# hediet/slideo

Hardware: AMD Instinct MI355X
Metric: frames/sec matched (1080p vs 500-page ORB set) (higher is better)
Workload: dtype u8

## Files before the change

### slideo_amd/csrc/capi_runtime.hip

```cpp
#include "runtime.hpp"
#include <chrono>

using namespace slideo;

namespace slideo {

namespace {
std::string g_create_error;
std::mutex g_err_mutex;
}

void check_launch(const char* what) {
    hipError_t e = hipGetLastError();
    if (e != hipSuccess) fail(SLIDEO_ERR_HIP, "launch of %s failed: %s", what, hipGetErrorString(e));
}

GeomEntry& geom_for(slideo_matcher* m, int w, int h) {
    for (auto& g : m->geoms) if (g->w == w && g->h == h) return *g;
    if (w < 1 || h < 1 || w > MAX_DIM || h > MAX_DIM)
        fail(SLIDEO_ERR_UNSUPPORTED, "image size %dx%d outside 1..%d", w, h, MAX_DIM);
    auto e = std::make_unique<GeomEntry>();
    e->w = w; e->h = h;
    std::vector<uint32_t> tab;
    build_pyr_geom(w, h, m->cfg, e->g, tab);
// ... 224 lines not shown
    const PyrGeom& g = geom_for(m, f.w, f.h).g;
    const uint32_t kpcap = kp_cap_for(m, g);
    const bool async = allow_async && m->async_submit && !knn_unit_is_valu(m) &&
                       (int64_t)n * kpcap < ((int64_t)1 << 30) &&
                       (kpcap >= (uint32_t)c.nfeatures + 1024u || kpcap >= (uint32_t)std::max(g.cand_per_frame, 1));
    S.timed = prof; S.u_in = f; S.u_mask = mask_pyr; S.u_async = async;
    if (m->orb_chain && m->last_orb_ev && m->last_orb_ev != S.ev_orb) HIP_CHECK(hipStreamWaitEvent(st, m->last_orb_ev, 0));
    if (prof) HIP_CHECK(hipEventRecord(S.ev[0], st));
    orb_stage1(m, S, f, n, false, async ? kpcap : 0xFFFFFFFFu, mask_pyr);
    uint32_t qtot, qplan;
    if (async) {
        qtot = (uint32_t)n * kpcap;
        qplan = (uint32_t)n * std::min<uint32_t>(kpcap, (uint32_t)c.nfeatures);
        S.orb.qtot = qtot; S.orb.max_count = kpcap;
    } else {
        orb_wait_info(m, S);
        qtot = qplan = S.orb.qtot;
    }
    knn_plan_unit(m, S, n, (int64_t)f.w * f.h, qplan, qtot);
    S.d_votes.reserve(std::max<size_t>((size_t)qtot * c.knn_k * sizeof(uint2), 16));
    S.d_gpts.reserve(std::max<size_t>((size_t)qtot * c.knn_k * sizeof(float4), 16));
    S.d_gmask.reserve(std::max<size_t>((size_t)qtot * c.knn_k, 16));
    S.d_fcs.reserve((size_t)n * sizeof(FrameCands));
    S.d_verdicts.reserve((size_t)n * sizeof(slideo_verdict));
    S.d_pairs.reserve((size_t)n * MAXR * sizeof(PairDesc) + 64);
    S.h_out.reserve((size_t)n * (sizeof(slideo_verdict) + sizeof(FrameCands)) + 64);
    orb_stage2(m, S, f.w, f.h, async);
    HIP_CHECK(hipEventRecord(S.ev_orb, st));
    m->last_orb_ev = S.ev_orb;
    VerifyParams vp = make_vp(c);
    vp.rng_len = m->rng_len;
    HIP_CHECK(hipMemsetAsync(S.d_fcs.p, 0, (size_t)n * sizeof(FrameCands), st));
    if (prof) HIP_CHECK(hipEventRecord(S.ev[1], st));
    if (qtot > 0) unit_knn(m, S, n, qplan, qtot, async, prof);
    unit_verify(m, S, vp, f, n, qtot);
}

void unit_collect(slideo_matcher* m, Slot& S, slideo_verdict* out_host) {
    const int n = S.n;
    HIP_CHECK(hipStreamSynchronize(S.st));
    S.busy = false;
    const uint8_t* ho = S.h_out.as<uint8_t>();
    const size_t tail = (size_t)n * (sizeof(slideo_verdict) + sizeof(FrameCands));
    uint32_t fl, info[2];
    std::memcpy(&fl, ho + tail, 4);
    std::memcpy(info, ho + tail + 4, 8);
    if (S.u_async) {
        if (fl & 1u) fail(SLIDEO_ERR_HIP, "internal: FAST candidate list overflow");
        if (fl & 8u) {
            S.u_rerun = true;
            unit_submit(m, S, S.u_in, n, S.u_mask, false);
            unit_collect(m, S, out_host);
            return;
        }
        S.orb.qtot = info[0]; S.orb.max_count = info[1];
    }
    const uint32_t qtot = S.orb.qtot;
    if (fl & 4u) {
        const uint32_t cap = 1u << 26;
        if (m->rng_len >= cap) fail(SLIDEO_ERR_CAPACITY, "RANSAC sample schedule exceeded %u pre-drawn RNG outputs", m->rng_len);
        HIP_CHECK(hipDeviceSynchronize());
        upload_rng_stream(m, (uint32_t)std::min<uint64_t>((uint64_t)m->rng_len * 4, cap));
        S.u_rerun = true;
        unit_submit(m, S, S.u_in, n, S.u_mask, false);
        unit_collect(m, S, out_host);
        return;
    }
    if (S.timed) {
// ... 1078 lines not shown
```

### slideo_amd/csrc/capi_taps.hip

```cpp
#include "runtime.hpp"

using namespace slideo;

extern "C" {


int32_t slideo_orb_bgr8(slideo_matcher* m, const uint8_t* bgr, int32_t width, int32_t height, int32_t stride_bytes,
                        slideo_keypoint* kp, uint8_t* desc32, int32_t capacity, int32_t* n_out) {
    if (!m) return SLIDEO_ERR_INVALID_ARG;
    API_TRY
    if (!bgr || !n_out) fail(SLIDEO_ERR_INVALID_ARG, "null image/n_out");
    FrameSrc img = FrameSrc::image(bgr, width, height, stride_bytes);
    validate_frames(img);
    HIP_CHECK(hipSetDevice(m->device));
    require_idle(m);
    Slot& S = m->slots[0];
    hipStream_t st = S.st;
    const uint8_t* mask_pyr = (m->fs.mask.set && width == m->fs.mask.w && height == m->fs.mask.h) ? frame_mask_for(m, width, height) : nullptr;
    run_orb(m, S, stage_frames(m, S, img, 0, 1), 1, false, false, mask_pyr);
    const uint32_t q = S.orb.qtot;
    *n_out = (int32_t)q;
    if ((int64_t)q > capacity) fail(SLIDEO_ERR_CAPACITY, "%u keypoints, capacity %d", q, capacity);
    if (q) {
        if (kp) HIP_CHECK(hipMemcpyAsync(kp, S.d_kp.p, (size_t)q * sizeof(slideo_keypoint), hipMemcpyDeviceToHost, st));
// ... 119 lines not shown
    Slot& S = m->slots[0];
    hipStream_t st = S.st;
    const size_t tail = (size_t)n * (sizeof(slideo_verdict) + sizeof(FrameCands));
    for (;;) {
        S.knn.shared = false; S.gate.on = false; S.u_set = m->cur_set; S.u_rerun = false;
        const DevFrames f = stage_frames(m, S, src, 0, n);
        S.timed = false; S.u_in = f; S.u_mask = nullptr; S.u_async = false;
        S.orb.qofs = qofs; S.orb.qtot = qtot; S.orb.max_count = mx; S.orb.nframes = n;
        S.d_kp.reserve(std::max<size_t>((size_t)qtot * sizeof(slideo_keypoint), 16));
        S.d_desc.reserve(std::max<size_t>((size_t)qtot * 32, 32));
        S.d_qofs.reserve((size_t)(n + 1) * 4 + 16); S.d_info.reserve(64); S.d_flags.reserve(16);
        S.h_info.reserve((size_t)(n + 1) * 4 + 16);
        uint32_t* hq = S.h_info.as<uint32_t>();
        std::memcpy(hq, qofs.data(), (size_t)(n + 1) * 4);
        hq[n + 1] = qtot; hq[n + 2] = mx;
        if (qtot > 0) {
            HIP_CHECK(hipMemcpyAsync(S.d_kp.p, kp, (size_t)qtot * sizeof(slideo_keypoint), hipMemcpyHostToDevice, st));
            HIP_CHECK(hipMemcpyAsync(S.d_desc.p, desc32, (size_t)qtot * 32, hipMemcpyHostToDevice, st));
        }
        HIP_CHECK(hipMemcpyAsync(S.d_qofs.p, hq, (size_t)(n + 1) * 4, hipMemcpyHostToDevice, st));
        HIP_CHECK(hipMemcpyAsync(S.d_info.p, hq + n + 1, 8, hipMemcpyHostToDevice, st));
        HIP_CHECK(hipMemsetAsync(S.d_flags.p, 0, 16, st));
        knn_plan_unit(m, S, n, (int64_t)f.w * f.h, qtot, qtot);
        S.d_votes.reserve(std::max<size_t>((size_t)qtot * c.knn_k * sizeof(uint2), 16));
        S.d_gpts.reserve(std::max<size_t>((size_t)qtot * c.knn_k * sizeof(float4), 16));
        S.d_gmask.reserve(std::max<size_t>((size_t)qtot * c.knn_k, 16));
        S.d_fcs.reserve((size_t)n * sizeof(FrameCands));
        S.d_verdicts.reserve((size_t)n * sizeof(slideo_verdict));
        S.d_pairs.reserve((size_t)n * MAXR * sizeof(PairDesc) + 64);
        S.h_out.reserve(tail + 64);
        HIP_CHECK(hipMemsetAsync(S.d_fcs.p, 0, (size_t)n * sizeof(FrameCands), st));
        VerifyParams vp = make_vp(c);
        vp.rng_len = m->rng_len;
        if (qtot > 0) unit_knn(m, S, n, qtot, qtot, false, false);
        unit_verify(m, S, vp, f, n, qtot);
        HIP_CHECK(hipStreamSynchronize(st));
        S.busy = false;
        uint32_t fl;
        std::memcpy(&fl, S.h_out.as<uint8_t>() + tail, 4);
        if (!(fl & 4u)) break;
        const uint32_t cap = 1u << 26;
        if (m->rng_len >= cap) fail(SLIDEO_ERR_CAPACITY, "RANSAC sample schedule exceeded %u pre-drawn RNG outputs", m->rng_len);
        HIP_CHECK(hipDeviceSynchronize());
        upload_rng_stream(m, (uint32_t)std::min<uint64_t>((uint64_t)m->rng_len * 4, cap));
    }
    const uint8_t* ho = S.h_out.as<uint8_t>();
    std::memcpy(verdicts_out, ho, (size_t)n * sizeof(slideo_verdict));
    m->last_fcs.resize((size_t)n);
    std::memcpy(m->last_fcs.data(), ho + (size_t)n * sizeof(slideo_verdict), (size_t)n * sizeof(FrameCands));
    API_CATCH(m)
}

int32_t slideo_yuv420_to_bgr8(slideo_matcher* m, const uint8_t* frame, int32_t width, int32_t height, const slideo_yuv420_layout* layout,
                              uint8_t* bgr_out, int64_t out_capacity) {
    if (!m) return SLIDEO_ERR_INVALID_ARG;
    API_TRY
    if (!frame || !bgr_out) fail(SLIDEO_ERR_INVALID_ARG, "null frame/bgr_out");
    FrameSrc img = FrameSrc::yuv420(frame, false, width, height, layout, -1);
    img.describe(m->fs);
    img.levels = false;
    validate_frames(img);
    const size_t fb = (size_t)width * height * 3;
    if ((int64_t)fb > out_capacity) fail(SLIDEO_ERR_CAPACITY, "the BGR image needs %zu bytes", fb);
    tap_staged(m, img, bgr_out, (int64_t)fb);
    API_CATCH(m)
}

}
// ... 1 lines not shown
```

### slideo_amd/csrc/orb.hip.h

```cpp
#pragma once
#include <limits.h>
#include <hip/hip_runtime.h>
#include <stdint.h>

#include "geom.h"
#include "types.h"
#include "cv_math.hip.h"

namespace slideo {

__global__ __launch_bounds__(256) void gray_kernel(const uint8_t* __restrict__ frames, int64_t frame_stride,
                                                   int stride, uint8_t* __restrict__ pyr, int64_t pyr_frame_bytes,
                                                   int w, int h, int pitch, int aligned4, GrayCoef gc) {
    const uint32_t half = 1u << (gc.shift - 1);
    auto gray_of = [&](uint32_t b, uint32_t g, uint32_t r) { return (__umul24(b, gc.cb) + __umul24(g, gc.cg) + __umul24(r, gc.cr) + half) >> gc.shift; };
    const int x = (blockIdx.x * 256 + threadIdx.x) * 4;
    const int y = blockIdx.y;
    if (x >= w) return;
    const uint8_t* src = frames + (int64_t)blockIdx.z * frame_stride + (int64_t)y * stride + (int64_t)x * 3;
    uint8_t* dst = pyr + (int64_t)blockIdx.z * pyr_frame_bytes + (int64_t)y * pitch + x;
    if (aligned4 && x + 3 < w) {
        const uint32_t* s = reinterpret_cast<const uint32_t*>(src);
        uint32_t a = s[0], b = s[1], c = s[2];
        uint32_t g0 = gray_of(a & 255, (a >> 8) & 255, (a >> 16) & 255);
// ... 63 lines not shown
#pragma unroll
            for (int i = 0; i < 4; ++i) {
                const int xo = xe[i] & 0xffff, cx1 = xe[i] >> 16, cx0 = 256 - cx1;
                const int xo1 = min(xo + 1, src.w - 1);
                uint32_t h0 = (uint32_t)cx0 * r0[xo] + (uint32_t)cx1 * r0[xo1];
                uint32_t h1 = (uint32_t)cx0 * r1[xo] + (uint32_t)cx1 * r1[xo1];
                v[i] = (uint32_t)cy0 * h0 + (uint32_t)cy1 * h1 + (1u << 15);
            }
        }
        const uint32_t outv = __builtin_amdgcn_perm(__builtin_amdgcn_perm(v[3], v[2], 0x0c0c0602u),
                                                    __builtin_amdgcn_perm(v[1], v[0], 0x0c0c0602u), 0x05040100u);
        uint8_t* d = base + dst.ofs + __umul24(y, dst.pitch) + x0;
        if (nx == 4) *reinterpret_cast<uint32_t*>(d) = outv;
        else for (int i = 0; i < nx; ++i) d[i] = (uint8_t)(outv >> (8 * i));
    }
}

__global__ __launch_bounds__(256) void resize_quad_kernel(uint8_t* __restrict__ pyr, int64_t pyr_frame_bytes,
                                                          LevelGeom src, LevelGeom dst,
                                                          const uint32_t* __restrict__ lin_tab, int nxq, uint32_t nxq_magic) {
    const uint32_t t = blockIdx.x * 256 + threadIdx.x;
    const uint32_t yg = nxq_magic ? __umulhi(t, nxq_magic) : t;
    const uint32_t y0 = yg * 4u;
    if ((int)y0 >= dst.h) return;
    const uint32_t q = t - __umul24(yg, (uint32_t)nxq);
    const uint8_t* __restrict__ sbase = pyr + (int64_t)blockIdx.z * pyr_frame_bytes + src.ofs;
    uint8_t* __restrict__ dbase = pyr + (int64_t)blockIdx.z * pyr_frame_bytes + dst.ofs;
    const uint4 sel4 = reinterpret_cast<const uint4*>(lin_tab + dst.xsel_ofs)[q];
    const uint4 cp4 = reinterpret_cast<const uint4*>(lin_tab + dst.xctab_ofs)[q];
    const uint32_t xs = lin_tab[dst.xs_ofs + q];
    const uint4 ye4 = *reinterpret_cast<const uint4*>(lin_tab + dst.ytab_ofs + y0);
    const uint32_t ye[4] = {ye4.x, ye4.y, ye4.z, ye4.w};
    const uint32_t sel[4] = {sel4.x, sel4.y, sel4.z, sel4.w}, cp[4] = {cp4.x, cp4.y, cp4.z, cp4.w};
    uint2 a[4], b[4];
#pragma unroll
    for (int r = 0; r < 4; ++r) {
        const uint32_t yo = ye[r] & 0xffffu;
        const uint32_t o0 = __umul24(yo, (uint32_t)src.pitch) + xs;
        const uint32_t o1 = __umul24(min(yo + 1u, (uint32_t)(src.h - 1)), (uint32_t)src.pitch) + xs;
        {
            const uint32_t sh = (xs & 3u) * 8u;
            uint32_t w0[3], w1[3];
            __builtin_memcpy(w0, sbase + (o0 & ~3u), 12);
            __builtin_memcpy(w1, sbase + (o1 & ~3u), 12);
            a[r] = make_uint2(__builtin_amdgcn_alignbit(w0[1], w0[0], sh), __builtin_amdgcn_alignbit(w0[2], w0[1], sh));
            b[r] = make_uint2(__builtin_amdgcn_alignbit(w1[1], w1[0], sh), __builtin_amdgcn_alignbit(w1[2], w1[1], sh));
        }
    }
    const uint32_t dofs = __umul24(y0, (uint32_t)dst.pitch) + 4u * q;
#pragma unroll
    for (int r = 0; r < 4; ++r) {
        const uint32_t cy1 = ye[r] >> 16, cy0 = 256u - cy1;
        uint32_t v[4];
#pragma unroll
        for (int i = 0; i < 4; ++i) {
            const uint32_t ta = __builtin_amdgcn_perm(a[r].y, a[r].x, sel[i]);
            const uint32_t tb = __builtin_amdgcn_perm(b[r].y, b[r].x, sel[i]);
            v[i] = __umul24(cy0, dot2_u16(ta, cp[i])) + (__umul24(cy1, dot2_u16(tb, cp[i])) + (1u << 15));
        }
        const uint32_t outv = __builtin_amdgcn_perm(__builtin_amdgcn_perm(v[3], v[2], 0x0c0c0602u),
                                                    __builtin_amdgcn_perm(v[1], v[0], 0x0c0c0602u), 0x05040100u);
        if ((int)(y0 + r) < dst.h) *reinterpret_cast<uint32_t*>(dbase + (dofs + (uint32_t)r * (uint32_t)dst.pitch)) = outv;
    }
}

__device__ __forceinline__ bool run9(uint32_t m) {
    m |= m << 16;
    m &= m >> 1; m &= m >> 2; m &= m >> 4; m &= m >> 1;
    return m != 0;
}

__device__ __forceinline__ int level_of_tile(const PyrGeom& g, int tile, bool blur) {
    int l = 0;
    for (int i = 1; i < g.nlevels; ++i) {
        int t0 = blur ? g.lv[i].btile0 : g.lv[i].ftile0;
        int n = blur ? g.lv[i].btx * g.lv[i].bty : g.lv[i].ftx * g.lv[i].fty;
        if (n > 0 && tile >= t0) l = i;
    }
    return l;
}

constexpr int FAST_SW = FAST_TW + 2, FAST_SH = FAST_TH + 2;
constexpr int FAST_XO = 4;
constexpr int FAST_RW = FAST_TW + 14, FAST_RH = FAST_TH + 8;
static_assert(FAST_SW == 128 && FAST_RW % 4 == 0 && (FAST_RW / 4) % 2 == 1 && FAST_RW >= FAST_SW + FAST_XO + 3, "fast_kernel maps one score row onto two wave-widths");

typedef short fast_s2 __attribute__((ext_vector_type(2)));
typedef unsigned short fast_us2 __attribute__((ext_vector_type(2)));
__device__ __forceinline__ fast_s2 fast_swap(fast_s2 a) { return __builtin_shufflevector(a, a, 1, 0); }

#ifndef FAST_TPB_V
#define FAST_TPB_V 8
#endif
constexpr int FAST_TPB = FAST_TPB_V;
constexpr int FAST_STAGE_CAP = 128;
// ... 873 lines not shown
```

### slideo_amd/csrc/runtime.hpp

```cpp
#pragma once
#include <hip/hip_runtime.h>

#include <algorithm>
#include <cmath>
#include <cstdlib>
#include <functional>
#include <map>
#include <memory>
#include <mutex>
#include <string>
#include <vector>

#include "common.h"
#include "frame_settings.h"
#include "geom.h"
#include "slideo_amd.h"
#include "types.h"

namespace slideo {

#ifndef SLIDEO_NSLOTS
#define SLIDEO_NSLOTS 4
#endif
constexpr int NSLOTS = SLIDEO_NSLOTS;
// ... 339 lines not shown
    float max_error = std::sqrt((255.0f * 255.0f * 3.0f) * (float)n);
    return 1.0f - (float)e / max_error;
}
uint8_t* stage_for_upload(slideo_matcher* m, Slot& S, size_t bytes);
void tap_staged(slideo_matcher* m, const FrameSrc& img, uint8_t* out, int64_t ob);
void analyse_pages(slideo_matcher* m, int n_pages, const uint8_t* const* data, const int32_t* width, const int32_t* height, const int32_t* stride_bytes,
                   std::vector<HostPage>& out, uint64_t progress_base, uint64_t progress_total);
void append_page(slideo_matcher* m, const HostPage& pg);

void orb_stage_init(slideo_matcher* m);
void orb_geom_init(slideo_matcher* m, GeomEntry& e, const std::vector<uint32_t>& lin_tab);
void orb_stage1(slideo_matcher* m, Slot& S, const DevFrames& f, int n, bool with_blur = false, uint32_t kp_cap = 0xFFFFFFFFu,
                const uint8_t* mask_pyr = nullptr);
void orb_wait_info(slideo_matcher* m, Slot& S);
void orb_stage2(slideo_matcher* m, Slot& S, int w, int h, bool by_capacity = false);
void run_orb(slideo_matcher* m, Slot& S, const DevFrames& f, int n, bool keep_host_qofs, bool with_blur = false, const uint8_t* mask_pyr = nullptr);
void frame_mask_build(slideo_matcher* m, const uint8_t* mask, int w, int h, int stride, DevBuf& out);
const uint8_t* frame_mask_for(const slideo_matcher* m, int w, int h);
void orb_launch_gray(const slideo_matcher* m, const uint8_t* frames_dev, int64_t frame_stride, int stride, uint8_t* gray, int64_t gframe, int w, int h,
                     int pitch, int n, hipStream_t st);
void orb_launch_scan(const uint32_t* counts, int n, uint32_t* qofs, uint32_t* info, hipStream_t st);
void launch_reduce(slideo_matcher* m, const uint8_t* src, int64_t src_fs, int stride, int w, int h, int dw, int dh, int n, uint8_t* dst,
                   hipStream_t st);
void launch_rectify(const FrameRegion& R, const uint8_t* src, int64_t src_fs, int stride, int n, uint8_t* dst, hipStream_t st);
void frame_region_classify(FrameRegion& R);
void launch_yuv420_to_bgr(const YuvDesc& desc, const uint8_t* src, int64_t src_fs, const slideo_yuv420_layout& L, int w, int h, int n, uint8_t* dst, hipStream_t st,
                          const uint32_t* transfer_tab = nullptr);
void launch_pixels_to_bgr(int format, const uint8_t* src, int64_t src_fs, int stride, int w, int h, int n, uint8_t* dst, hipStream_t st);
void launch_levels(slideo_matcher* m, const uint8_t* src, int64_t src_fs, int src_stride, uint8_t* dst, int64_t dst_fs, int dst_stride, int w, int h,
                   int n, hipStream_t st);

void knn_build_index(slideo_matcher* m, const std::vector<uint8_t>& train, int64_t M);
void knn_plan_unit(slideo_matcher* m, Slot& S, int n, int64_t frame_pixels, uint32_t qplan, uint32_t qtot);
void unit_knn(slideo_matcher* m, Slot& S, int n, uint32_t qplan, uint32_t qtot, bool async, bool prof);
bool knn_unit_is_valu(const slideo_matcher* m);
void knn_expand_operand(const uint32_t* t, int nt, int nt_pad, const int32_t* perm, uint4* tx, hipStream_t st);
int knn_operand_rows(int nt);
OperandLayout knn_operand_layout();
std::vector<int32_t> knn_tile_order(int ntiles);
void l2_prepare(slideo_matcher::L2Set& L, const uint8_t* t, int nt, hipStream_t st);
void l2_query(slideo_matcher* m, slideo_matcher::L2Set& L, const uint8_t* q_dev, int nq, int k, hipStream_t st, Slot& S, bool timed,
              DevBuf* keys = nullptr, DevBuf* pend = nullptr, float prune_tol = 0.f);
void l2_lists_to_keys(slideo_matcher* m, Slot& S, const DevBuf& lists, int kq, uint32_t qtot, bool lowe, hipStream_t st);

void verify_stage_init(slideo_matcher* m);
VerifyParams make_vp(const slideo_config& c);
void unit_verify(slideo_matcher* m, Slot& S, const VerifyParams& vp, const DevFrames& f, int n, uint32_t qtot);
void run_small(slideo_matcher* m, const DevFrames& imgs, int n, hipStream_t st, int* sw = nullptr, int* sh = nullptr);
void run_small_into(slideo_matcher* m, const DevFrames& imgs, int n, DevBuf& dst, hipStream_t st, int* sw = nullptr, int* sh = nullptr);
void launch_ssd(const uint8_t* a, int64_t a_stride, const uint8_t* b, int64_t b_stride, int64_t bytes, unsigned long long* ssd, int n, hipStream_t st);

int page_set_create(slideo_matcher* m, int n, const int32_t* pages);
const PageSet* page_set_of(const slideo_matcher* m, int set);
void page_set_check_mode(const slideo_matcher* m);

void gate_release(slideo_matcher* m);
inline void gate_state_reset(slideo_matcher* m) { m->gate = slideo_matcher::GateState{}; }
inline size_t gate_small_budget(const slideo_matcher* m) {
    const size_t small = (size_t)m->cfg.small_area * 3 + 64;
    const size_t settle = m->fs.settle_similarity > 0.f ? small + 256 + 32 : 0;
    const size_t M = (size_t)m->fs.gate_memory;
    const size_t memory = M > 0 ? 8 * M + 8 : 0;
    const size_t anchor = m->fs.gate_ref == SLIDEO_GATE_ANCHOR ? small + 128 + 32 + (size_t)GATE_ANCHOR_MAX_UNIT * 8 + settle + memory : 0;
    if (!(m->fs.direct_t > 0.f)) return small + anchor;
    const size_t look = 2 * small + 128 + m->pages.size() * 8 + 64 + anchor;
    return m->fs.direct_scope == SLIDEO_DIRECT_VALID ? look + m->pages.size() * 8 : look;
}
inline size_t gate_memory_budget(const slideo_matcher* m) {
    const size_t M = m->fs.gate_ref == SLIDEO_GATE_ANCHOR ? (size_t)m->fs.gate_memory : 0;
    return M > 0 ? (M + 64) * ((size_t)m->cfg.small_area * 3 + 64 + 128) + 2048 : 0;
}
void gate_check(const slideo_matcher::GateState& g, const FrameSrc& src);
void gate_prime(slideo_matcher* m, FrameSrc src, hipStream_t user_stream);
void gate_state_read(slideo_matcher* m, hipEvent_t behind, size_t sb, uint8_t* anchor, uint8_t* prev, uint32_t* d);
void gate_state_write(slideo_matcher* m, size_t sb, const uint8_t* anchor, const uint8_t* prev, const uint32_t* d, hipStream_t st);
inline void gate_chain_receive(slideo_matcher* m, hipStream_t st) {
    if (!m->gate_receive) return;
    const std::function<void(hipStream_t)> f = std::move(m->gate_receive);
    m->gate_receive = nullptr;
    f(st);
// ... 64 lines not shown
```

### slideo_amd/csrc/stage_knn.hip

```cpp
#include "runtime.hpp"
#include "knn.hip.h"
#include "knn_tile.hip.h"
#include "knn_l2.hip.h"
#include "knn_lsh.hip.h"

using namespace slideo;

namespace slideo {

int knn_operand_rows(int nt) { return cdiv(std::max(nt, 1), KT_ST_ROWS) * KT_ST_ROWS; }
OperandLayout knn_operand_layout() { return OperandLayout{KT_ST_ROWS, KT_SIDE_U32, KT_PAD_NORM}; }

void knn_expand_operand(const uint32_t* t, int nt, int nt_pad, const int32_t* perm, uint4* tx, hipStream_t st) {
    knn_tile_expand_kernel<<<cdiv(nt_pad * 8, 256), 256, 0, st>>>(t, nt, nt_pad, perm, tx);
    check_launch("knn_tile_expand_kernel");
}

std::vector<int32_t> knn_tile_order(int ntiles) {
    std::vector<int32_t> order((size_t)ntiles);
    for (int i = 0; i < ntiles; ++i) order[i] = i;
    uint64_t st_ = 0x9E3779B97F4A7C15ull;
    for (int i = ntiles - 1; i > 0; --i) {
        st_ = st_ * 6364136223846793005ull + 1442695040888963407ull;
        std::swap(order[i], order[(int)((st_ >> 33) % (uint64_t)(i + 1))]);
// ... 156 lines not shown
    const uint4* tx = op.tx.as<uint4>(); const uint32_t* side = op.side.as<uint32_t>(); const float4* nminh = op.bound.as<float4>();
    const int nt_pad = knn_operand_rows(p.nt);
    uint32_t *keys = S.d_keys.as<uint32_t>(), *pend = S.d_knn_pend.as<uint32_t>();
    unsigned long long* const clk = m->profiling ? m->d_clk.as<unsigned long long>() : nullptr;
    if (lsh)
        knn_tile2_lsh_kernel<<<grid, KT_THREADS, 0, st>>>(q_dev, nq, tx, side, nminh, nt_pad, p.per_seg, keys, pend, prune_tol, nq_dev, *lsh);
    else if (p.engine == 2)
        knn_tile4_kernel<<<grid, KT_THREADS, 0, st>>>(q_dev, nq, tx, side, nminh, nt_pad, p.per_seg, keys, pend, prune_tol, nq_dev);
    else if (p.shape == SHAPE_T2W12)
        knn_tile2w12_kernel<<<grid, KT_WAVES12 * 64, 0, st>>>(q_dev, nq, tx, side, nminh, nt_pad, p.per_seg, keys, pend, prune_tol, nq_dev, clk);
    else
        knn_tile2_kernel<<<grid, KT_THREADS, p.lds_pad, st>>>(q_dev, nq, tx, side, nminh, nt_pad, p.per_seg, keys, pend, prune_tol, nq_dev, clk);
    check_launch(lsh ? "knn_tile2_lsh_kernel" : "knn_tile_kernel");
    if (p.nseg > 1) {
        knn_merge_kernel<KLIST><<<cdiv(p.nq_all, KNN_BLOCK), KNN_BLOCK, 0, st>>>(keys, nq, p.nseg, nq_dev);
        check_launch("knn_merge_kernel");
    }
}

static void run_knn(slideo_matcher* m, Slot& S, const KnnPlan& p, const uint32_t* q_dev, int nq, const uint32_t* t, const SearchOperand& op,
                    float prune_tol, const uint32_t* nq_dev = nullptr) {
    if (nq <= 0 && !nq_dev) return;
    if ((int64_t)p.nt >= ((int64_t)1 << KNN_KEY_SHIFT)) fail(SLIDEO_ERR_UNSUPPORTED, "train set of %d rows exceeds %d", p.nt, 1 << KNN_KEY_SHIFT);
    if (p.engine != 1) { knn_launch_tiles(m, S, p, q_dev, nq, op, prune_tol, nq_dev); return; }
    if (nq_dev) fail(SLIDEO_ERR_STATE, "internal: the VALU kNN engine needs the query count on the host");
    knn_hamming_kernel<KLIST><<<dim3(p.qblocks, p.nseg), KNN_BLOCK, 0, S.st>>>(q_dev, nq, t, p.nt, p.per_seg, S.d_keys.as<uint32_t>());
    check_launch("knn_hamming_kernel");
    if (p.nseg > 1) {
        knn_merge_kernel<KLIST><<<p.qblocks, KNN_BLOCK, 0, S.st>>>(S.d_keys.as<uint32_t>(), nq, p.nseg);
        check_launch("knn_merge_kernel");
    }
}

void unit_knn(slideo_matcher* m, Slot& S, int n, uint32_t qplan, uint32_t qtot, bool async, bool prof) {
    const slideo_config& c = m->cfg;
    hipStream_t st = S.st;
    const KnnPlan& p = S.knn;
    const PageSet* ps = page_set_of(m, S.u_set);
    const SearchOperand& op = ps ? ps->op : m->train_op;
    const uint32_t* nqd = async ? S.d_qofs.as<uint32_t>() + n : nullptr;
    const float prune = (m->knn_exact_lists || m->cfg.ratio_test > 0.f) ? 0.f : std::max(m->cfg.vote_tolerance, 1.0f);
    if (c.matcher == 1 && (m->lsh_gather || knn_unit_is_valu(m))) {
        knn_lsh_kernel<KLIST><<<cdiv((int)std::max(qtot, 1u), 4), 256, 0, st>>>(m->lsh.dev, S.d_desc.as<uint32_t>(), (int)qtot, m->d_train.as<uint32_t>(),
                                                                               S.d_keys.as<uint32_t>(), nqd);
        check_launch("knn_lsh_kernel");
    } else if (c.matcher == 1) {
        S.d_qkeys.reserve(std::max<size_t>((size_t)qtot * c.lsh_tables * 2, 64));
        lsh_query_keys_kernel<<<cdiv((int)std::max(qtot, 1u), 256), 256, 0, st>>>(m->lsh.dev.p, S.d_desc.as<uint32_t>(), (int)qtot, S.d_qkeys.as<uint16_t>(), nqd);
        check_launch("lsh_query_keys_kernel");
        const KtLshCtx ctx{m->lsh.dev.keys, S.d_qkeys.as<uint16_t>(), c.lsh_tables, c.lsh_multi_probe};
        knn_launch_tiles(m, S, p, S.d_desc.as<uint32_t>(), (int)qplan, op, prune, nqd, &ctx);
    } else
        run_knn(m, S, p, S.d_desc.as<uint32_t>(), (int)qplan, ps ? nullptr : m->d_train.as<uint32_t>(), op, prune, nqd);
    if (prof) HIP_CHECK(hipEventRecord(S.ev[2], st));
    if (p.dedup) {
        knn_expand_dups_kernel<KLIST><<<cdiv((int)std::max(qtot, 1u), KNN_BLOCK), KNN_BLOCK, 0, st>>>(
            S.d_keys.as<uint32_t>(), (int)qtot, (ps ? ps->d_grp_next : m->d_grp_next).as<int32_t>(), nqd);
        check_launch("knn_expand_dups_kernel");
    }
}

void knn_build_index(slideo_matcher* m, const std::vector<uint8_t>& train, int64_t M) {
    m->d_train.reserve(std::max<size_t>(train.size(), 64) + 64);
    HIP_CHECK(hipMemcpy(m->d_train.p, train.data(), train.size(), hipMemcpyHostToDevice));
    std::vector<int32_t> order((size_t)M), grp_next((size_t)M, -1), urow;
    for (int64_t i = 0; i < M; ++i) order[i] = (int32_t)i;
    m->Mu = M;
    if (m->cfg.matcher == 1) build_lsh_set(m->cfg, train.data(), (int)M, m->lsh, m->stream);
    if (m->knn_dedup && m->cfg.matcher == 0) {
        const uint64_t* t64 = reinterpret_cast<const uint64_t*>(train.data());
        auto less = [&](int32_t a, int32_t b) {
            const uint64_t* x = t64 + (size_t)a * 4; const uint64_t* y = t64 + (size_t)b * 4;
            for (int j = 0; j < 4; ++j) if (x[j] != y[j]) return x[j] < y[j];
            return a < b;
        };
        std::sort(order.begin(), order.end(), less);
        std::vector<uint8_t> head((size_t)M, 1);
        for (int64_t i = 1; i < M; ++i)
            if (std::memcmp(t64 + (size_t)order[i - 1] * 4, t64 + (size_t)order[i] * 4, 32) == 0) { grp_next[order[i - 1]] = order[i]; head[order[i]] = 0; }
        for (int64_t i = 0; i < M; ++i) if (head[i]) urow.push_back((int32_t)i);
        m->Mu = (int64_t)urow.size();
    }
    m->d_grp_next.reserve(grp_next.size() * 4 + 16);
    HIP_CHECK(hipMemcpy(m->d_grp_next.p, grp_next.data(), grp_next.size() * 4, hipMemcpyHostToDevice));
    if (m->Mu < M) {
        std::vector<uint8_t> utrain((size_t)m->Mu * 32);
        for (int64_t i = 0; i < m->Mu; ++i) std::memcpy(utrain.data() + (size_t)i * 32, train.data() + (size_t)urow[i] * 32, 32);
        m->d_utrain.reserve(utrain.size() + 64);
        HIP_CHECK(hipMemcpy(m->d_utrain.p, utrain.data(), utrain.size(), hipMemcpyHostToDevice));
        prepare_train_bits(utrain.data(), m->d_utrain.as<uint32_t>(), (int)m->Mu, m->train_op, m->stream, urow.data(), &m->h_uorder);
        m->h_urow.swap(urow);
    } else {
// ... 185 lines not shown
```

### slideo_amd/csrc/stage_sift.hip

```cpp
#include "runtime.hpp"
#include "sift.hip.h"

using namespace slideo;

namespace slideo {

static SiftGeom sift_geom(int w, int h) {
    SiftGeom g{};
    g.w = w; g.h = h;
    int bw = 2 * w, bh = 2 * h;
    g.n_oct = std::max(0, (int)std::lrint(std::log((double)std::min(bw, bh)) / std::log(2.) - 2) + 1);
    if (g.n_oct > SIFT_MAX_OCT) g.n_oct = SIFT_MAX_OCT;
    int64_t go = 0, dofs = 0;
    for (int o = 0; o < g.n_oct; ++o) {
        g.ow[o] = bw; g.oh[o] = bh; g.g_ofs[o] = go; g.d_ofs[o] = dofs;
        go += (int64_t)bw * bh * (SIFT_NL + 3); dofs += (int64_t)bw * bh * (SIFT_NL + 2);
        bw /= 2; bh /= 2;
        if (bw < 1 || bh < 1) { g.n_oct = o + 1; break; }
    }
    g.g_frame = go; g.d_frame = dofs;
    return g;
}

static SiftTaps sift_taps(double sigma) {
// ... 215 lines not shown
    S.orb.qtot = qtot; S.orb.max_count = mx; S.orb.nframes = n;
    S.knn.nt = (int)m->M;
    S.d_qofs.reserve((size_t)(n + 1) * 4 + 16); S.d_info.reserve(16); S.d_flags.reserve(16);
    S.h_info.reserve((size_t)(n + 1) * 4 + 16);
    uint32_t* hq = S.h_info.as<uint32_t>();
    std::memcpy(hq, S.orb.qofs.data(), (size_t)(n + 1) * 4);
    hq[n + 1] = qtot; hq[n + 2] = mx;
    HIP_CHECK(hipMemcpyAsync(S.d_qofs.p, hq, (size_t)(n + 1) * 4, hipMemcpyHostToDevice, st));
    HIP_CHECK(hipMemcpyAsync(S.d_info.p, hq + n + 1, 8, hipMemcpyHostToDevice, st));
    HIP_CHECK(hipMemsetAsync(S.d_flags.p, 0, 16, st));
    const bool lowe = m->sift_ratio > 0.f;
    const int kq = lowe ? 2 : c.knn_k;
    S.d_keys.reserve(std::max<size_t>((size_t)qtot * KLIST * 4, 64));
    S.d_votes.reserve(std::max<size_t>((size_t)qtot * kq * sizeof(uint2), 16));
    S.d_gpts.reserve(std::max<size_t>((size_t)qtot * kq * sizeof(float4), 16));
    S.d_gmask.reserve(std::max<size_t>((size_t)qtot * kq, 16));
    S.d_fcs.reserve((size_t)n * sizeof(FrameCands));
    S.d_verdicts.reserve((size_t)n * sizeof(slideo_verdict));
    S.d_pairs.reserve((size_t)n * MAXR * sizeof(PairDesc) + 64);
    S.h_out.reserve((size_t)n * (sizeof(slideo_verdict) + sizeof(FrameCands)) + 64);
    HIP_CHECK(hipMemsetAsync(S.d_fcs.p, 0, (size_t)n * sizeof(FrameCands), st));
    HIP_CHECK(hipEventRecord(m->sift_ev, st));
    m->sift_ev_set = true;
    if (prof) HIP_CHECK(hipEventRecord(S.ev[1], st));
    if (qtot > 0) {
        l2_query(m, m->l2, S.d_desc.as<uint8_t>(), (int)qtot, kq, st, S, false, &S.d_blur, &S.d_knn_pend, !lowe ? c.vote_tolerance : 0.f);
        l2_lists_to_keys(m, S, S.d_blur, kq, qtot, lowe, st);
    }
    if (prof) HIP_CHECK(hipEventRecord(S.ev[2], st));
    VerifyParams vp = make_vp(c);
    vp.rng_len = m->rng_len;
    if (lowe) { vp.k = 2; vp.ratio = 1.f; }
    else { vp.k = kq; vp.ratio = 0.f; vp.tol = 1.5f; }
    unit_verify(m, S, vp, f, n, qtot);
}

void add_pages_sift(slideo_matcher* m, Slot& S, const DevFrames& pages, int cnt) {
    sift_check_cfg(&m->sift_cfg, pages.w, pages.h);
    std::vector<uint32_t> counts((size_t)cnt, 0);
    int64_t cap = sift_unit_capacity(m, cnt), rows = 0;
    for (int attempt = 0; attempt < 2; ++attempt) {
        S.d_kp.reserve(std::max<size_t>((size_t)cap * sizeof(slideo_keypoint), 64));
        S.d_desc.reserve(std::max<size_t>((size_t)cap * 128, 128));
        rows = sift_batch(m, pages.p, cnt, pages.w, pages.h, pages.stride, pages.frame_stride, m->sift_cfg, 0, cap, S.d_kp.as<slideo_keypoint>(),
                          S.d_desc.as<uint8_t>(), counts.data(), S.st);
        if (rows <= cap) break;
        cap = rows;
    }
    HIP_CHECK(hipStreamSynchronize(S.st));
    S.orb.qofs.assign((size_t)cnt + 1, 0);
    for (int i = 0; i < cnt; ++i) S.orb.qofs[i + 1] = S.orb.qofs[i] + counts[i];
    S.orb.qtot = (uint32_t)rows; S.orb.nframes = cnt;
}

}

extern "C" {

void slideo_sift_config_default(slideo_sift_config* c) {
    if (!c) return;
    c->nfeatures = 0; c->n_octave_layers = 3; c->contrast_threshold = 0.04; c->edge_threshold = 10; c->sigma = 1.6;
}

int32_t slideo_matcher_use_sift(slideo_matcher* m, const slideo_sift_config* cfg, float ratio) {
    if (!m) return SLIDEO_ERR_INVALID_ARG;
    API_TRY
    if (!m->pages.empty() || m->finalized) fail(SLIDEO_ERR_STATE, "slideo_matcher_use_sift must precede the first page");
// ... 92 lines not shown
```

### slideo_amd/csrc/stage_verify.hip

```cpp
#include "runtime.hpp"
#include "verify.hip.h"
#include "homography.hip.h"

using namespace slideo;

namespace slideo {

VerifyParams make_vp(const slideo_config& c) {
    VerifyParams v{};
    v.k = c.knn_k; v.klist = KLIST; v.max_cand = c.max_candidate_pages; v.max_rated = c.max_rated;
    v.tol = c.vote_tolerance; v.min_similarity = c.min_similarity; v.ratio = c.ratio_test;
    v.thr = c.ransac_threshold; v.conf = c.ransac_confidence; v.min_rating = c.min_rating;
    v.min_rating_ratio = c.min_rating_ratio; v.max_iters = c.ransac_max_iters; v.refine_iters = c.refine_iters;
    v.model = c.verify_model; v.verdict_rule = c.verdict_rule;
    v.sched_window = env_long("SLIDEO_RANSAC_WINDOW", 1) != 0;
    return v;
}

void run_small(slideo_matcher* m, const DevFrames& imgs, int n, hipStream_t st, int* sw, int* sh) {
    run_small_into(m, imgs, n, m->d_small, st, sw, sh);
}

void run_small_into(slideo_matcher* m, const DevFrames& imgs, int n, DevBuf& dst, hipStream_t st, int* sw_out, int* sh_out) {
    int ac = area_class_for(m, imgs.w, imgs.h);
    upload_area(m);
    const AreaGeom& ag = m->area_geoms[ac];
    const int sw = ag.dw, sh = ag.dh;
    if (sw_out) { *sw_out = sw; *sh_out = sh; }
    dst.reserve((size_t)n * sw * sh * 3);
    int tiles = cdiv(sw, SM_TW) * cdiv(sh, SM_TH);
    small_image_kernel<<<dim3(tiles, n), 256, 0, st>>>(ag, m->d_area_taps.as<AreaTap>(), m->d_area_idx.as<int32_t>(), imgs.p,
                                                       imgs.frame_stride, imgs.stride, dst.as<uint8_t>(), (int64_t)sw * sh * 3);
    check_launch("small_image_kernel");
}

void launch_ssd(const uint8_t* a, int64_t a_stride, const uint8_t* b, int64_t b_stride, int64_t bytes, unsigned long long* ssd, int n, hipStream_t st) {
    ssd_kernel<<<n, 256, 0, st>>>(a, a_stride, b, b_stride, bytes, ssd);
    check_launch("ssd_kernel");
}

void unit_verify(slideo_matcher* m, Slot& S, const VerifyParams& vp, const DevFrames& f, int n, uint32_t qtot) {
    const slideo_config& c = m->cfg;
    hipStream_t st = S.st;
    const bool prof = m->profiling;
    const int P = (int)m->pages.size();
    uint32_t* flags = S.d_flags.as<uint32_t>();
    if (qtot > 0) {
        const size_t lds = (size_t)P * 4 + (((size_t)P + 15) & ~(size_t)15) + (size_t)c.max_candidate_pages * 256 * 4;
        vote_kernel<<<n, 256, lds, st>>>(vp, S.d_keys.as<uint32_t>(), S.d_qofs.as<uint32_t>(), m->d_train_page.as<int32_t>(), P,
                                         S.d_fcs.as<FrameCands>(), S.d_votes.as<uint2>());
        check_launch("vote_kernel");
        if (c.verify_model == 1) {
            const long tail_env = env_long("SLIDEO_RH_TAIL_ROUNDS", 256);
            const uint32_t tail_rounds = (uint32_t)(tail_env < 1 ? 0xFFFFFFFFu : tail_env);
            const uint32_t round_cap = c.ocv.hdlt ? tail_rounds : 0xFFFFFFFFu;
            S.d_tail.reserve((size_t)c.max_candidate_pages * n * 4 + 16);
            auto launch_h = [&](auto small_tag, auto large_tag, int hdlt) {
                small_tag<<<dim3(c.max_candidate_pages, n), 64, ransac_h_lds_bytes(RANSAC_SMALL_PTS, hdlt), st>>>(
                    vp, S.d_qofs.as<uint32_t>(), S.d_kp.as<slideo_keypoint>(), m->d_page_xy.as<float2>(), S.d_votes.as<uint2>(),
                    m->d_rng.as<uint32_t>(), S.d_fcs.as<FrameCands>(), S.d_gpts.as<float4>(), S.d_gmask.as<uint8_t>(), flags, round_cap,
                    S.d_tail.as<uint32_t>(), flags + 1);
                check_launch("ransac_h_kernel (small)");
                large_tag<<<dim3(c.max_candidate_pages, n), 64, ransac_h_lds_bytes(RANSAC_LDS_PTS, hdlt), st>>>(
                    vp, S.d_qofs.as<uint32_t>(), S.d_kp.as<slideo_keypoint>(), m->d_page_xy.as<float2>(), S.d_votes.as<uint2>(),
                    m->d_rng.as<uint32_t>(), S.d_fcs.as<FrameCands>(), S.d_gpts.as<float4>(), S.d_gmask.as<uint8_t>(), flags, round_cap,
                    S.d_tail.as<uint32_t>(), flags + 1);
                check_launch("ransac_h_kernel (large)");
            };
            auto launch_tail = [&](auto tail_tag) {
                const int blocks = std::min(RANSAC_H_TAIL_BLOCKS, c.max_candidate_pages * n);
                tail_tag<<<blocks, 64 * RANSAC_H_TAIL_WAVES, ransac_h_tail_lds_bytes(RANSAC_H_TAIL_WAVES), st>>>(
                    vp, S.d_qofs.as<uint32_t>(), S.d_kp.as<slideo_keypoint>(), m->d_page_xy.as<float2>(), S.d_votes.as<uint2>(),
                    m->d_rng.as<uint32_t>(), S.d_fcs.as<FrameCands>(), S.d_gpts.as<float4>(), S.d_gmask.as<uint8_t>(), flags,
                    S.d_tail.as<uint32_t>(), flags + 1, flags + 2);
                check_launch("ransac_h_tail_kernel");
            };
            if (c.ocv.hdlt == 2) {
                launch_h(&ransac_h_kernel<RANSAC_SMALL_PTS, 0, 2>, &ransac_h_kernel<RANSAC_LDS_PTS, RANSAC_SMALL_PTS + 1, 2>, 2);
                if (round_cap != 0xFFFFFFFFu) launch_tail(&ransac_h_tail_kernel<2, RANSAC_H_TAIL_WAVES>);
            } else if (c.ocv.hdlt == 1) {
                launch_h(&ransac_h_kernel<RANSAC_SMALL_PTS, 0, 1>, &ransac_h_kernel<RANSAC_LDS_PTS, RANSAC_SMALL_PTS + 1, 1>, 1);
                if (round_cap != 0xFFFFFFFFu) launch_tail(&ransac_h_tail_kernel<1, RANSAC_H_TAIL_WAVES>);
// ... 100 lines not shown
```

### slideo_amd/csrc/verify.hip.h

```cpp
#pragma once
#include <hip/hip_runtime.h>
#include <stdint.h>

#include <type_traits>

#include "geom.h"
#include "types.h"

namespace slideo {


__global__ __launch_bounds__(256) void vote_kernel(VerifyParams vp, const uint32_t* __restrict__ keys,
                                                   const uint32_t* __restrict__ qofs,
                                                   const int32_t* __restrict__ train_page, int npages,
                                                   FrameCands* __restrict__ fcs, uint2* __restrict__ votes) {
    extern __shared__ __attribute__((aligned(16))) uint8_t smem[];
    uint32_t* counts = reinterpret_cast<uint32_t*>(smem);
    uint8_t* rank = smem + (size_t)npages * 4;
    uint32_t* runcnt = reinterpret_cast<uint32_t*>(smem + (size_t)npages * 4 + (((size_t)npages + 15) & ~(size_t)15));
    __shared__ unsigned long long red[4];
    __shared__ int32_t s_page[MAXC], s_count[MAXC], s_ofs[MAXC];

    const int f = blockIdx.x, tid = threadIdx.x, lane = tid & 63, wave = tid >> 6;
    const uint32_t q0 = qofs[f], n = qofs[f + 1] - q0;
    const int k = vp.k;
    FrameCands& fc = fcs[f];
    for (int i = tid; i < npages; i += 256) { counts[i] = 0; rank[i] = 0xFF; }
    __syncthreads();
    const uint32_t runq = (n + 255) / 256;
    const uint32_t qa = min(n, (uint32_t)tid * runq), qb = min(n, qa + runq);
    auto for_each_vote = [&](auto&& fn) {
        for (uint32_t q = qa; q < qb; ++q) {
            const uint4* kq4 = reinterpret_cast<const uint4*>(keys + (size_t)(q0 + q) * VOTE_KLIST);
            uint32_t key[VOTE_KLIST];
#pragma unroll
            for (int i = 0; i < VOTE_KLIST / 4; ++i) { const uint4 v = kq4[i]; key[4 * i] = v.x; key[4 * i + 1] = v.y; key[4 * i + 2] = v.z; key[4 * i + 3] = v.w; }
            if (vp.ratio > 0.f) {
                if (k >= 2 && key[0] != KNN_EMPTY && key[1] != KNN_EMPTY &&
                    (float)(key[0] >> KNN_KEY_SHIFT) < vp.ratio * (float)(key[1] >> KNN_KEY_SHIFT))
                    fn(q, key[0] & KNN_IDX_MASK);
                continue;
            }
            const float lim = (float)(key[0] >> KNN_KEY_SHIFT) * vp.tol;
#pragma unroll
            for (int r = 0; r < VOTE_KLIST; ++r) {
                const bool pass = r < k && key[r] != KNN_EMPTY && (float)(key[r] >> KNN_KEY_SHIFT) < lim;
                if (!pass) break;
                fn(q, key[r] & KNN_IDX_MASK);
            }
        }
    };
    for_each_vote([&](uint32_t, uint32_t t) { atomicAdd(&counts[train_page[t]], 1u); });
    __syncthreads();
    int nc = 0;
    for (int round = 0; round < vp.max_cand; ++round) {
        unsigned long long best = 0;
        for (int p = tid; p < npages; p += 256) {
            uint32_t c = counts[p];
            if (c && rank[p] == 0xFF) {
                unsigned long long comp = ((unsigned long long)c << 32) | (0xFFFFFFFFu - (uint32_t)p);
                best = comp > best ? comp : best;
            }
        }
#pragma unroll
        for (int d = 32; d > 0; d >>= 1) {
            unsigned long long o = __shfl_xor(best, d);
            best = o > best ? o : best;
        }
        if (lane == 0) red[wave] = best;
        __syncthreads();
        best = red[0];
        for (int w = 1; w < 4; ++w) best = red[w] > best ? red[w] : best;
        __syncthreads();
        if (best == 0) break;
        int p = (int)(0xFFFFFFFFu - (uint32_t)(best & 0xFFFFFFFFu));
        if (tid == 0) { s_page[nc] = p; s_count[nc] = (int32_t)(best >> 32); rank[p] = (uint8_t)nc; }
        ++nc;
        __syncthreads();
    }
    if (tid == 0) {
        int o = 0;
// ... 1044 lines not shown
```

Before: 24140.

## Fold duplicate-descriptor expansion into vote kernel and reuse resize row passes

Drops the separate knn_expand_dups kernel. The vote kernel now walks the duplicate-group chains (grp_next) inline, merging equal-distance duplicate train indices in index order while voting. The point is to save a launch and a full read/write pass over the KNN key list. Separately, the quad resize kernel now detects across the wavefront when a row's top source row equals the previous row's bottom row. In that case it reuses the horizontal pass and skips the load, and the vertical blend becomes a single dot2. The cost is more complex, branchy chain-walking logic in vote_kernel.

```diff
diff --git a/profiles/summarize_pmc_dispatches.py b/profiles/summarize_pmc_dispatches.py
--- /dev/null
+++ b/profiles/summarize_pmc_dispatches.py
@@ -0,0 +1,19 @@
+#!/usr/bin/env python3
+import sqlite3, sys, collections
+c = sqlite3.connect(sys.argv[1])
+acc = collections.defaultdict(lambda: collections.defaultdict(lambda: collections.defaultdict(float)))
+dur = {}
+for name, cn, val, d, did in c.execute("select kernel_name, counter_name, value, duration, dispatch_id from counters_collection"):
+    k = name.split("(")[0][:56]
+    acc[k][cn][did] += val
+    dur[(k, did)] = d
+want = ("fast_kernel", "blur_f32", "describe_blurred", "resize_quad", "resize_kernel", "gray_kernel", "reproject", "ransac_kernel", "vote_kernel",
+        "knn_expand_dups", "sort_kernel", "compact_kernel", "rate_kernel", "verdict_kernel", "knn_tile")
+for k in sorted(acc):
+    if not any(w in k for w in want):
+        continue
+    ds = [d for (kk, _), d in dur.items() if kk == k]
+    print("%s: dispatches %d, total %.1f us" % (k, len(ds), sum(ds) / 1e3))
+    for cn in sorted(acc[k]):
+        v = sorted(acc[k][cn].values())
+        print("    %-16s sum %14.0f   per dispatch min %12.0f max %12.0f   largest three %s" % (cn, sum(v), v[0], v[-1], " ".join("%.0f" % x for x in v[-3:])))
diff --git a/slideo_amd/csrc/capi_runtime.hip b/slideo_amd/csrc/capi_runtime.hip
--- a/slideo_amd/csrc/capi_runtime.hip
+++ b/slideo_amd/csrc/capi_runtime.hip
@@ -280,8 +280,8 @@
     vp.rng_len = m->rng_len;
     HIP_CHECK(hipMemsetAsync(S.d_fcs.p, 0, (size_t)n * sizeof(FrameCands), st));
     if (prof) HIP_CHECK(hipEventRecord(S.ev[1], st));
-    if (qtot > 0) unit_knn(m, S, n, qplan, qtot, async, prof);
-    unit_verify(m, S, vp, f, n, qtot);
+    const int32_t* chain = qtot > 0 ? unit_knn(m, S, n, qplan, qtot, async, prof) : nullptr;
+    unit_verify(m, S, vp, f, n, qtot, chain);
 }
 
 void unit_collect(slideo_matcher* m, Slot& S, slideo_verdict* out_host) {
diff --git a/slideo_amd/csrc/capi_taps.hip b/slideo_amd/csrc/capi_taps.hip
--- a/slideo_amd/csrc/capi_taps.hip
+++ b/slideo_amd/csrc/capi_taps.hip
@@ -175,8 +175,8 @@
         HIP_CHECK(hipMemsetAsync(S.d_fcs.p, 0, (size_t)n * sizeof(FrameCands), st));
         VerifyParams vp = make_vp(c);
         vp.rng_len = m->rng_len;
-        if (qtot > 0) unit_knn(m, S, n, qtot, qtot, false, false);
-        unit_verify(m, S, vp, f, n, qtot);
+        const int32_t* chain = qtot > 0 ? unit_knn(m, S, n, qtot, qtot, false, false) : nullptr;
+        unit_verify(m, S, vp, f, n, qtot, chain);
         HIP_CHECK(hipStreamSynchronize(st));
         S.busy = false;
         uint32_t fl;
diff --git a/slideo_amd/csrc/orb.hip.h b/slideo_amd/csrc/orb.hip.h
--- a/slideo_amd/csrc/orb.hip.h
+++ b/slideo_amd/csrc/orb.hip.h
@@ -119,35 +119,44 @@
     const uint4 ye4 = *reinterpret_cast<const uint4*>(lin_tab + dst.ytab_ofs + y0);
     const uint32_t ye[4] = {ye4.x, ye4.y, ye4.z, ye4.w};
     const uint32_t sel[4] = {sel4.x, sel4.y, sel4.z, sel4.w}, cp[4] = {cp4.x, cp4.y, cp4.z, cp4.w};
-    uint2 a[4], b[4];
+    uint32_t ra[4], rb[4];
+#pragma unroll
+    for (int r = 0; r < 4; ++r) { ra[r] = ye[r] & 0xffffu; rb[r] = min(ra[r] + 1u, (uint32_t)(src.h - 1)); }
+    bool taken[4] = {false, false, false, false};
+#pragma unroll
+    for (int r = 1; r < 4; ++r) taken[r] = __builtin_amdgcn_ballot_w64(ra[r] != rb[r - 1]) == 0;
+    uint32_t wa[4][3], wb[4][3];
 #pragma unroll
     for (int r = 0; r < 4; ++r) {
-        const uint32_t yo = ye[r] & 0xffffu;
-        const uint32_t o0 = __umul24(yo, (uint32_t)src.pitch) + xs;
-        const uint32_t o1 = __umul24(min(yo + 1u, (uint32_t)(src.h - 1)), (uint32_t)src.pitch) + xs;
-        {
-            const uint32_t sh = (xs & 3u) * 8u;
-            uint32_t w0[3], w1[3];
-            __builtin_memcpy(w0, sbase + (o0 & ~3u), 12);
-            __builtin_memcpy(w1, sbase + (o1 & ~3u), 12);
-            a[r] = make_uint2(__builtin_amdgcn_alignbit(w0[1], w0[0], sh), __builtin_amdgcn_alignbit(w0[2], w0[1], sh));
-            b[r] = make_uint2(__builtin_amdgcn_alignbit(w1[1], w1[0], sh), __builtin_amdgcn_alignbit(w1[2], w1[1], sh));
-        }
-    }
+        if (!taken[r]) __builtin_memcpy(wa[r], sbase + ((__umul24(ra[r], (uint32_t)src.pitch) + xs) & ~3u), 12);
+        __builtin_memcpy(wb[r], sbase + ((__umul24(rb[r], (uint32_t)src.pitch) + xs) & ~3u), 12);
+    }
+    const uint32_t sh = (xs & 3u) * 8u;
+    auto hpass = [&](const uint32_t (&w)[3], uint32_t (&h)[4]) {
+        const uint32_t lo = __builtin_amdgcn_alignbit(w[1], w[0], sh), hi = __builtin_amdgcn_alignbit(w[2], w[1], sh);
+#pragma unroll
+        for (int i = 0; i < 4; ++i) h[i] = dot2_u16(__builtin_amdgcn_perm(hi, lo, sel[i]), cp[i]);
+    };
     const uint32_t dofs = __umul24(y0, (uint32_t)dst.pitch) + 4u * q;
+    uint32_t h[2][4];
 #pragma unroll
     for (int r = 0; r < 4; ++r) {
-        const uint32_t cy1 = ye[r] >> 16, cy0 = 256u - cy1;
-        uint32_t v[4];
-#pragma unroll
-        for (int i = 0; i < 4; ++i) {
-            const uint32_t ta = __builtin_amdgcn_perm(a[r].y, a[r].x, sel[i]);
-            const uint32_t tb = __builtin_amdgcn_perm(b[r].y, b[r].x, sel[i]);
-            v[i] = __umul24(cy0, dot2_u16(ta, cp[i])) + (__umul24(cy1, dot2_u16(tb, cp[i])) + (1u << 15));
-        }
-        const uint32_t outv = __builtin_amdgcn_perm(__builtin_amdgcn_perm(v[3], v[2], 0x0c0c0602u),
-                                                    __builtin_amdgcn_perm(v[1], v[0], 0x0c0c0602u), 0x05040100u);
-        if ((int)(y0 + r) < dst.h) *reinterpret_cast<uint32_t*>(dbase + (dofs + (uint32_t)r * (uint32_t)dst.pitch)) = outv;
+        const uint32_t cyp = (ye[r] & 0xffff0000u) | (256u - (ye[r] >> 16));
+        auto out_row = [&](const uint32_t (&ha)[4], const uint32_t (&hb)[4]) {
+            uint32_t v[4];
+#pragma unroll
+            for (int i = 0; i < 4; ++i) v[i] = dot2_u16(ha[i] | (hb[i] << 16), cyp, 1u << 15);
+            const uint32_t outv = __builtin_amdgcn_perm(__builtin_amdgcn_perm(v[3], v[2], 0x0c0c0602u),
+                                                        __builtin_amdgcn_perm(v[1], v[0], 0x0c0c0602u), 0x05040100u);
+            if ((int)(y0 + r) < dst.h) *reinterpret_cast<uint32_t*>(dbase + (dofs + (uint32_t)r * (uint32_t)dst.pitch)) = outv;
+        };
+        hpass(wb[r], h[r & 1]);
+        if (taken[r]) out_row(h[(r - 1) & 1], h[r & 1]);
+        else {
+            uint32_t ha[4];
+            hpass(wa[r], ha);
+            out_row(ha, h[r & 1]);
+        }
     }
 }
 
diff --git a/slideo_amd/csrc/runtime.hpp b/slideo_amd/csrc/runtime.hpp
--- a/slideo_amd/csrc/runtime.hpp
+++ b/slideo_amd/csrc/runtime.hpp
@@ -395,7 +395,7 @@
 
 void knn_build_index(slideo_matcher* m, const std::vector<uint8_t>& train, int64_t M);
 void knn_plan_unit(slideo_matcher* m, Slot& S, int n, int64_t frame_pixels, uint32_t qplan, uint32_t qtot);
-void unit_knn(slideo_matcher* m, Slot& S, int n, uint32_t qplan, uint32_t qtot, bool async, bool prof);
+const int32_t* unit_knn(slideo_matcher* m, Slot& S, int n, uint32_t qplan, uint32_t qtot, bool async, bool prof);
 bool knn_unit_is_valu(const slideo_matcher* m);
 void knn_expand_operand(const uint32_t* t, int nt, int nt_pad, const int32_t* perm, uint4* tx, hipStream_t st);
 int knn_operand_rows(int nt);
@@ -408,7 +408,7 @@
 
 void verify_stage_init(slideo_matcher* m);
 VerifyParams make_vp(const slideo_config& c);
-void unit_verify(slideo_matcher* m, Slot& S, const VerifyParams& vp, const DevFrames& f, int n, uint32_t qtot);
+void unit_verify(slideo_matcher* m, Slot& S, const VerifyParams& vp, const DevFrames& f, int n, uint32_t qtot, const int32_t* grp_next);
 void run_small(slideo_matcher* m, const DevFrames& imgs, int n, hipStream_t st, int* sw = nullptr, int* sh = nullptr);
 void run_small_into(slideo_matcher* m, const DevFrames& imgs, int n, DevBuf& dst, hipStream_t st, int* sw = nullptr, int* sh = nullptr);
 void launch_ssd(const uint8_t* a, int64_t a_stride, const uint8_t* b, int64_t b_stride, int64_t bytes, unsigned long long* ssd, int n, hipStream_t st);
diff --git a/slideo_amd/csrc/stage_knn.hip b/slideo_amd/csrc/stage_knn.hip
--- a/slideo_amd/csrc/stage_knn.hip
+++ b/slideo_amd/csrc/stage_knn.hip
@@ -212,7 +212,7 @@
     }
 }
 
-void unit_knn(slideo_matcher* m, Slot& S, int n, uint32_t qplan, uint32_t qtot, bool async, bool prof) {
+const int32_t* unit_knn(slideo_matcher* m, Slot& S, int n, uint32_t qplan, uint32_t qtot, bool async, bool prof) {
     const slideo_config& c = m->cfg;
     hipStream_t st = S.st;
     const KnnPlan& p = S.knn;
@@ -233,11 +233,7 @@
     } else
         run_knn(m, S, p, S.d_desc.as<uint32_t>(), (int)qplan, ps ? nullptr : m->d_train.as<uint32_t>(), op, prune, nqd);
     if (prof) HIP_CHECK(hipEventRecord(S.ev[2], st));
-    if (p.dedup) {
-        knn_expand_dups_kernel<KLIST><<<cdiv((int)std::max(qtot, 1u), KNN_BLOCK), KNN_BLOCK, 0, st>>>(
-            S.d_keys.as<uint32_t>(), (int)qtot, (ps ? ps->d_grp_next : m->d_grp_next).as<int32_t>(), nqd);
-        check_launch("knn_expand_dups_kernel");
-    }
+    return p.dedup ? (ps ? ps->d_grp_next : m->d_grp_next).as<int32_t>() : nullptr;
 }
 
 void knn_build_index(slideo_matcher* m, const std::vector<uint8_t>& train, int64_t M) {
diff --git a/slideo_amd/csrc/stage_sift.hip b/slideo_amd/csrc/stage_sift.hip
--- a/slideo_amd/csrc/stage_sift.hip
+++ b/slideo_amd/csrc/stage_sift.hip
@@ -271,7 +271,7 @@
     vp.rng_len = m->rng_len;
     if (lowe) { vp.k = 2; vp.ratio = 1.f; }
     else { vp.k = kq; vp.ratio = 0.f; vp.tol = 1.5f; }
-    unit_verify(m, S, vp, f, n, qtot);
+    unit_verify(m, S, vp, f, n, qtot, nullptr);
 }
 
 void add_pages_sift(slideo_matcher* m, Slot& S, const DevFrames& pages, int cnt) {
diff --git a/slideo_amd/csrc/stage_verify.hip b/slideo_amd/csrc/stage_verify.hip
--- a/slideo_amd/csrc/stage_verify.hip
+++ b/slideo_amd/csrc/stage_verify.hip
@@ -39,7 +39,7 @@
     check_launch("ssd_kernel");
 }
 
-void unit_verify(slideo_matcher* m, Slot& S, const VerifyParams& vp, const DevFrames& f, int n, uint32_t qtot) {
+void unit_verify(slideo_matcher* m, Slot& S, const VerifyParams& vp, const DevFrames& f, int n, uint32_t qtot, const int32_t* grp_next) {
     const slideo_config& c = m->cfg;
     hipStream_t st = S.st;
     const bool prof = m->profiling;
@@ -47,7 +47,7 @@
     uint32_t* flags = S.d_flags.as<uint32_t>();
     if (qtot > 0) {
         const size_t lds = (size_t)P * 4 + (((size_t)P + 15) & ~(size_t)15) + (size_t)c.max_candidate_pages * 256 * 4;
-        vote_kernel<<<n, 256, lds, st>>>(vp, S.d_keys.as<uint32_t>(), S.d_qofs.as<uint32_t>(), m->d_train_page.as<int32_t>(), P,
+        vote_kernel<<<n, 256, lds, st>>>(vp, S.d_keys.as<uint32_t>(), grp_next, S.d_qofs.as<uint32_t>(), m->d_train_page.as<int32_t>(), P,
                                          S.d_fcs.as<FrameCands>(), S.d_votes.as<uint2>());
         check_launch("vote_kernel");
         if (c.verify_model == 1) {
diff --git a/slideo_amd/csrc/verify.hip.h b/slideo_amd/csrc/verify.hip.h
--- a/slideo_amd/csrc/verify.hip.h
+++ b/slideo_amd/csrc/verify.hip.h
@@ -10,7 +10,7 @@
 namespace slideo {
 
 
-__global__ __launch_bounds__(256) void vote_kernel(VerifyParams vp, const uint32_t* __restrict__ keys,
+__global__ __launch_bounds__(256) void vote_kernel(VerifyParams vp, const uint32_t* __restrict__ keys, const int32_t* __restrict__ grp_next,
                                                    const uint32_t* __restrict__ qofs,
                                                    const int32_t* __restrict__ train_page, int npages,
                                                    FrameCands* __restrict__ fcs, uint2* __restrict__ votes) {
@@ -36,17 +36,63 @@
 #pragma unroll
             for (int i = 0; i < VOTE_KLIST / 4; ++i) { const uint4 v = kq4[i]; key[4 * i] = v.x; key[4 * i + 1] = v.y; key[4 * i + 2] = v.z; key[4 * i + 3] = v.w; }
             if (vp.ratio > 0.f) {
-                if (k >= 2 && key[0] != KNN_EMPTY && key[1] != KNN_EMPTY &&
-                    (float)(key[0] >> KNN_KEY_SHIFT) < vp.ratio * (float)(key[1] >> KNN_KEY_SHIFT))
-                    fn(q, key[0] & KNN_IDX_MASK);
+                if (k >= 2 && key[0] != KNN_EMPTY) {
+                    const bool dup = grp_next && grp_next[key[0] & KNN_IDX_MASK] >= 0;
+                    const uint32_t second = dup ? key[0] : key[1];
+                    if (second != KNN_EMPTY && (float)(key[0] >> KNN_KEY_SHIFT) < vp.ratio * (float)(second >> KNN_KEY_SHIFT))
+                        fn(q, key[0] & KNN_IDX_MASK);
+                }
                 continue;
             }
             const float lim = (float)(key[0] >> KNN_KEY_SHIFT) * vp.tol;
+            int np = 0;
+            uint32_t heads = 0;
 #pragma unroll
             for (int r = 0; r < VOTE_KLIST; ++r) {
                 const bool pass = r < k && key[r] != KNN_EMPTY && (float)(key[r] >> KNN_KEY_SHIFT) < lim;
                 if (!pass) break;
-                fn(q, key[r] & KNN_IDX_MASK);
+                if (grp_next) heads |= grp_next[key[r] & KNN_IDX_MASK] >= 0 ? 1u << r : 0u;
+                ++np;
+            }
+            if (!heads) {
+#pragma unroll
+                for (int r = 0; r < VOTE_KLIST; ++r) {
+                    if (r >= np) break;
+                    fn(q, key[r] & KNN_IDX_MASK);
+                }
+                continue;
+            }
+            const uint32_t* kq = keys + (size_t)(q0 + q) * VOTE_KLIST;
+            int left = k;
+            for (int i0 = 0; i0 < np && left > 0;) {
+                uint32_t hkey = kq[i0];
+                const uint32_t dk = hkey >> KNN_KEY_SHIFT;
+                int ih = i0, ci = -1;
+                bool more = true;
+                uint32_t open = 0;
+                int32_t last = -1, crow = 0;
+                for (; left > 0; --left) {
+                    int32_t next = more ? (int32_t)(hkey & KNN_IDX_MASK) : INT32_MAX;
+                    int from = -1;
+                    for (uint32_t o = open; o; o &= o - 1) {
+                        const int i = __ffs((int)o) - 1;
+                        int32_t row = i == ci ? crow : (int32_t)(kq[i] & KNN_IDX_MASK);
+                        while (row >= 0 && row <= last) row = grp_next[row];
+                        if (row < 0) open &= ~(1u << i);
+                        else if (row < next) { next = row; from = i; }
+                    }
+                    if (next == INT32_MAX) break;
+                    fn(q, (uint32_t)next);
+                    last = next;
+                    if (from >= 0) { ci = from; crow = next; }
+                    else {
+                        open |= heads & (1u << ih);
+                        ++ih;
+                        more = ih < np;
+                        if (more) { hkey = kq[ih]; more = (hkey >> KNN_KEY_SHIFT) == dk; }
+                    }
+                }
+                i0 = ih;
             }
         }
     };
```

After: 23930. Within noise of the previous version (-0.9%).
